# NVlabs/UnseenObjectClustering

Hardware: AMD Instinct MI355X
Metric: frames/sec at 640x480 RGB-D, two-stage clustering (higher is better)
Workload: dtype f32; 1 GPU; configs[3] frames: full two-stage (crop-and-refine) segmentation of single 640x480 RGB-D frames; throughput schedule 3 streams x 4-frame launch sets (one frame at a time: `latency`); frame=640x480, seeds=100, iters=10, crop=224, total_frames=513, frames_per_gpu=513, collective=False, frames_in_flight_per_gpu=12, streams_per_gpu=3, frames_per_launch=4

## Files before the change

### include/uoc_hip.h

```cpp
#ifndef UOC_HIP_H
#define UOC_HIP_H

#include <stddef.h>
#include <stdint.h>

#ifdef __cplusplus
extern "C" {
#endif

#define UOC_OK 0
#define UOC_EINVAL (-22)
#define UOC_ENOMEM (-12)
#define UOC_EHIP (-5)
#define UOC_ENOENT (-2)
#define UOC_ETIMEDOUT (-110)

#define UOC_EMBED_DIM 64
#define UOC_MAX_SEEDS 128
#define UOC_METRIC_COSINE 0
#define UOC_METRIC_EUCLIDEAN 1

int uoc_version(void);
int uoc_is_dev_build(void);
unsigned long long uoc_config_fingerprint(void);
// ... 57 lines not shown

int uoc_net_create(uoc_net **out);
int uoc_net_create_mode(uoc_net **out, int mode);
int uoc_net_embed_dim(const uoc_net *net);
int uoc_net_destroy(uoc_net *net);
int uoc_net_load_param(uoc_net *net, const char *name, const float *host_data, size_t numel);
int uoc_net_finalize(uoc_net *net);
size_t uoc_net_workspace_bytes(const uoc_net *net, int B, int H, int W);
int uoc_net_set_split_precision(uoc_net *net, int on);
int uoc_net_forward(uoc_net *net, const float *d_rgb, const float *d_xyz, int B, int H, int W, float *d_embed,
                    void *d_ws, size_t ws_bytes, void *stream);

#define UOC_CONV_DIRECT 0
#define UOC_CONV_WINOGRAD4 4
#define UOC_CONV_WINOGRAD4_BF16X3 5
int uoc_conv2d_nhwc(const float *d_in, const float *d_w, const float *d_bias, const float *d_res, float *d_out,
                    int G, int B, int H, int W, int Cin, int Cout, int K, int stride, int dil, int pad, int relu,
                    void *stream);
int uoc_conv2d_nhwc_algo(const float *d_in, const float *d_w, const float *d_bias, const float *d_res, float *d_out,
                         int G, int B, int H, int W, int Cin, int Cout, int K, int stride, int dil, int pad, int relu,
                         int algo, void *stream);

int uoc_conv2d_tile_list(int algo, int32_t *out_pairs, int cap);
int uoc_conv2d_nhwc_tile(const float *d_in, const float *d_w, const float *d_bias, const float *d_res, float *d_out,
                         int G, int B, int H, int W, int Cin, int Cout, int K, int stride, int dil, int pad, int relu,
                         int algo, void *stream, int cfg, int bm);
int uoc_conv2d_tile_choice(int G, int B, int H, int W, int Cin, int Cout, int K, int stride, int dil, int algo,
                           int32_t *cfg, int32_t *bm, int32_t *family_bm);
int uoc_net_stem(const float *d_nchw, const float *h_w, const float *h_bias, const float *d_res, int G, int B, int H,
                 int W, int relu, float *d_out, void *stream);
int uoc_maxpool3x3s2_nhwc(const float *d_in, float *d_out, int n_img, int H, int W, int C, void *stream);
int uoc_head(const float *d_fa, const float *d_fb, float *d_embed, int B, int h, int w, int H, int W, int cat,
             void *stream);


typedef struct uoc_roi_table {
  int32_t K;
  int32_t label[128];
  int32_t box[128][4];
} uoc_roi_table;

size_t uoc_roi_workspace_bytes(void);

int uoc_prep_rgbd(const uint8_t *d_bgr, const uint16_t *d_depth_mm, int H, int W, float fx, float fy, float px,
                  float py, float mean_b, float mean_g, float mean_r, float *d_image, float *d_xyz, void *stream);

int uoc_filter_labels_depth(int32_t *d_labels, const float *d_z, long z_batch_stride, int B, int H, int W,
                            float threshold, void *d_ws, size_t ws_bytes, void *stream);

int uoc_roi_build(int32_t *d_labels, const float *d_z, int H, int W, float threshold, float pad_fraction,
                  uoc_roi_table *d_table, void *d_ws, size_t ws_bytes, void *stream);

int uoc_roi_crop(const float *d_rgb, const float *d_xyz, const int32_t *d_labels, int H, int W,
                 const uoc_roi_table *d_table, int K, int S, float *d_rgb_crops, float *d_xyz_crops,
                 float *d_mask_crops, void *stream);

int uoc_roi_match_stats(const int32_t *d_labels_crop, const float *d_mask_crops, const float *d_xyz_crops, int K,
                        int S, int32_t *d_keep, float *d_meanz, void *d_ws, size_t ws_bytes, void *stream);

int uoc_roi_paste(const int32_t *d_labels_crop, const uoc_roi_table *d_table, const int32_t *d_map,
                  const int32_t *d_order, int K, int S, int H, int W, int32_t *d_refined, void *stream);

int uoc_roi_match(const int32_t *d_labels_crop, const float *d_mask_crops, const float *d_xyz_crops,
                  const uoc_roi_table *d_table, int K, int S, int H, int W, int32_t *d_refined, int32_t *d_keep,
                  int32_t *d_plan, int32_t *d_status, void *d_ws, size_t ws_bytes, void *stream);

// ... 253 lines not shown
```

### unseenobjectclustering_amd/_native.py

```python
from __future__ import annotations

import ctypes
import os
from ctypes import c_char_p, c_float, c_int, c_int32, c_long, c_size_t, c_uint32, c_ulonglong, c_void_p, POINTER

from .build import LIB_PATH

_lib = None


class NativeError(RuntimeError):
    pass


P, I, F, Z, L, U = c_void_p, c_int, c_float, c_size_t, c_long, c_uint32
ABI = {
    "uoc_version": (I, []),
    "uoc_is_dev_build": (I, []),
    "uoc_config_fingerprint": (c_ulonglong, []),
    "uoc_shutdown": (I, []),
    "uoc_last_error": (c_char_p, []),
    "uoc_reload_env": (I, []),
    "uoc_ms_set_persistent_fps": (I, [I]),
    "uoc_ms_set_stream_ordering": (I, [I]),
# ... 1 lines not shown
    "uoc_ms_check": (I, [P]),
    "uoc_ms_workspace_bytes": (Z, [I, I, I]),
    "uoc_ms_select_seeds": (I, [P, I, I, I, P, P, P, P, Z, P]),
    "uoc_ms_select_seeds_from": (I, [P, I, I, I, I, P, P, P, P, Z, P]),
    "uoc_ms_hill_climb": (I, [P, I, I, P, I, F, I, P, Z, P]),
    "uoc_ms_seed_components": (I, [P, I, I, F, P, P, P]),
    "uoc_ms_assign": (I, [P, I, I, P, P, P, I, P, P, P, Z, P]),
    "uoc_ms_cluster": (I, [P, I, I, I, F, I, F, P, P, P, P, P, P, Z, P]),
    "uoc_ms_workspace_bytes_wide": (Z, [I, I, I, I]),
    "uoc_ms_cluster_wide": (I, [P, I, I, I, I, F, I, F, P, P, P, P, P, P, Z, P]),
    "uoc_ms_select_seeds_ex": (I, [P, I, I, I, I, P, P, P, I, P, Z, P]),
    "uoc_ms_hill_climb_ex": (I, [P, I, I, P, I, F, I, I, P, Z, P]),
    "uoc_ms_seed_components_ex": (I, [P, I, I, F, I, P, P, P]),
    "uoc_ms_assign_ex": (I, [P, I, I, P, P, P, I, I, P, P, P, Z, P]),
    "uoc_ms_cluster_ex": (I, [P, I, I, I, F, I, F, I, P, P, P, P, P, P, Z, P]),
    "uoc_ms_cluster_wide_ex": (I, [P, I, I, I, I, F, I, F, I, P, P, P, P, P, P, Z, P]),
    "uoc_net_create": (I, [POINTER(P)]),
    "uoc_net_create_mode": (I, [POINTER(P), I]),
    "uoc_net_embed_dim": (I, [P]),
    "uoc_net_destroy": (I, [P]),
    "uoc_net_load_param": (I, [P, c_char_p, P, Z]),
    "uoc_net_finalize": (I, [P]),
    "uoc_net_workspace_bytes": (Z, [P, I, I, I]),
    "uoc_net_set_split_precision": (I, [P, I]),
    "uoc_net_forward": (I, [P, P, P, I, I, I, P, P, Z, P]),
    "uoc_conv2d_nhwc": (I, [P, P, P, P, P, I, I, I, I, I, I, I, I, I, I, I, P]),
    "uoc_conv2d_nhwc_algo": (I, [P, P, P, P, P, I, I, I, I, I, I, I, I, I, I, I, I, P]),
    "uoc_conv2d_tile_list": (I, [I, P, I]),
    "uoc_conv2d_nhwc_tile": (I, [P, P, P, P, P, I, I, I, I, I, I, I, I, I, I, I, I, P, I, I]),
    "uoc_conv2d_tile_choice": (I, [I, I, I, I, I, I, I, I, I, I, P, P, P]),
    "uoc_net_stem": (I, [P, P, P, P, I, I, I, I, I, P, P]),
    "uoc_maxpool3x3s2_nhwc": (I, [P, P, I, I, I, I, P]),
    "uoc_head": (I, [P, P, P, I, I, I, I, I, I, P]),
    "uoc_roi_workspace_bytes": (Z, []),
    "uoc_prep_rgbd": (I, [P, P, I, I, F, F, F, F, F, F, F, P, P, P]),
    "uoc_filter_labels_depth": (I, [P, P, L, I, I, I, F, P, Z, P]),
    "uoc_roi_build": (I, [P, P, I, I, F, F, P, P, Z, P]),
    "uoc_roi_crop": (I, [P, P, P, I, I, P, I, I, P, P, P, P]),
    "uoc_roi_match_stats": (I, [P, P, P, I, I, P, P, P, Z, P]),
    "uoc_roi_paste": (I, [P, P, P, P, I, I, I, I, P, P]),
    "uoc_roi_match": (I, [P, P, P, P, I, I, I, I, P, P, P, P, P, Z, P]),
    "uoc_labels_to_u8": (I, [P, L, P, P, P]),
    "uoc_eval_workspace_bytes": (Z, [I, I]),
    "uoc_eval_pair_stats": (I, [P, P, I, I, I, P, P, Z, P]),
    "uoc_objects_workspace_bytes": (Z, [I, I, I]),
    "uoc_objects": (I, [P, P, P, I, I, I, I, I, P, P, P, P, L, P, P, Z, P]),
    "uoc_track_state_bytes": (Z, [I, I, I]),
    "uoc_track_workspace_bytes": (Z, [I]),
    "uoc_track_reset": (I, [P, I, I, I, I, P]),
    "uoc_track_step": (I, [P, I, I, I, I, I, P, P, P, P, P, Z, P]),
    "uoc_cc_workspace_bytes": (Z, [I, I, I]),
    "uoc_cc_split": (I, [P, I, I, I, I, I, I, P, P, P, P, Z, P]),
    "uoc_plane_workspace_bytes": (Z, [I, I, I, I]),
    "uoc_support_plane": (I, [P, P, I, I, I, I, I, U, P, P, P, P, Z, P]),
    "uoc_planes_workspace_bytes": (Z, [I, I, I, I, I]),
    "uoc_support_planes": (I, [P, P, I, I, I, I, I, I, I, I, U, P, P, P, P, P, P, Z, P]),
    "uoc_relations_workspace_bytes": (Z, [I, I, I]),
    "uoc_relations": (I, [P, P, I, I, I, I, I, I, P, P, P, Z, P]),
    "uoc_placement_workspace_bytes": (Z, [I, I, I, I]),
    "uoc_placement": (I, [P, P, P, I, I, I, I, I, I, I, I, I, P, I, P, P, P, P, P, P, P, Z, P]),
    "uoc_grasp_workspace_bytes": (Z, [I, I, I, I]),
    "uoc_grasp": (I, [P, P, I, I, P, I, I, I, I, I, I, I, P, P, P, Z, P]),
    "uoc_elevation_workspace_bytes": (Z, [I, I, I, I]),
    "uoc_elevation": (I, [P, P, P, I, I, I, I, I, I, I, I, P, I, P, P, P, P, P, P, P, P, P, Z, P]),
    "uoc_footprint_workspace_bytes": (Z, [I, I, I, I]),
    "uoc_footprint": (I, [P, P, P, P, I, I, P, I, P, I, I, P, P, P, P, Z, P]),
# ... 290 lines not shown
```

### unseenobjectclustering_amd/csrc/conv.h

```cpp
#pragma once
#include "common.h"

namespace uoc {

struct ConvParams {
  const float *in;
  const float *w;
  const float *bias;
  const float *res;
  float *out;
  int G, B, H, W, Cin, Ho, Wo, Cout;
  int KH, KW, stride, dil, pad, relu;
  int stem;
  int tune = 1;
  int prof_kc = -1;
  double prof_flops = 0.0;
  int prof_tag[4] = {0, 0, 0, 0};
};

int launch_conv(const ConvParams &p, hipStream_t st);
int conv_tile_list(int *out_pairs, int cap);
int conv_tile_choice(const ConvParams &p, int *cfg, int *bm, int *fam_bm);
int launch_conv_tile(const ConvParams &p, hipStream_t st, int cfg, int bm);

struct W4Tile {
  int bm, bn;
};
int wino4_tile_list(bool split, int *out_pairs, int cap);
void wino4_tile_choice(bool split, int NT, int Cout, int planes, int *bn, int *bm);
int wino4_split_tile_list(int *out_pairs, int cap);
void wino4_split_tile_choice(int NT, int Cout, int planes, int *bn, int *bm);
void wino4_pick_tile(const int (*tiles)[2], int n, int NT, int Cout, int planes, int &bm, int &bn);
int wino4_plane_grid(int NT, int Cout, int planes, int bm, int bn);

bool wino4_eligible(const ConvParams &p);
bool wino4_channels_ok(int Cin, int Cout);
size_t wino4_ws_floats(int G, int B, int H, int W, int d, int Cin, int Cout);
int wino4_num_tiles(int B, int H, int W, int d);
int launch_wino4_weights(const float *w, float *U, int G, int Cout, int Cin, hipStream_t st);
int launch_wino4_conv(const ConvParams &p, const float *U, float *ws, hipStream_t st, const unsigned short *U3 = nullptr,
                      const W4Tile *tile = nullptr);
int launch_wino4_split_weights(const float *U, unsigned short *U3, int G, int Cout, int Cin, hipStream_t st);
int launch_wino4_slice_split(const ConvParams &p0, int Bg, int b0, const unsigned short *U3, float *ws, hipStream_t st,
                             const W4Tile *tile = nullptr);
struct Wino4Geom;
int w4_stage_output(const ConvParams &p, const Wino4Geom &geo, const float *Mw, hipStream_t st);
long wino4_elem_blocks(long items);
int launch_nchw3_to_nhwc4(const float *in, float *out, int B, int H, int W, hipStream_t st);
int launch_maxpool3x3s2(const float *in, float *out, int n_img, int H, int W, int C, int Ho, int Wo, hipStream_t st);
int launch_head(const float *fa, const float *fb, float *embed, int B, int h, int w, int H, int W, int cat,
                hipStream_t st);

}
```

### unseenobjectclustering_amd/csrc/net.hip

```cpp
#include <map>
#include <mutex>
#include <string>
#include <vector>

#include "conv.h"

#include <stdlib.h>

namespace uoc {

struct ConvLayer {
  std::string conv, bn;
  int Cin, Cout, K, stride, dil, pad, relu;
  bool has_bn, has_bias, stem;
  float *d_w = nullptr, *d_b = nullptr;
  float *d_U4 = nullptr;
  unsigned short *d_U3 = nullptr;
  size_t w_per_group = 0;
};

struct Block {
  int conv1, conv2, down;
};

// ... 438 lines not shown
int uoc_conv2d_nhwc_algo(const float *d_in, const float *d_w, const float *d_bias, const float *d_res, float *d_out, int G,
                         int B, int H, int W, int Cin, int Cout, int K, int stride, int dil, int pad, int relu, int algo,
                         void *stream) {
  return conv2d_entry(d_in, d_w, d_bias, d_res, d_out, G, B, H, W, Cin, Cout, K, stride, dil, pad, relu, algo, stream, nullptr);
}

int uoc_conv2d_nhwc_tile(const float *d_in, const float *d_w, const float *d_bias, const float *d_res, float *d_out, int G,
                         int B, int H, int W, int Cin, int Cout, int K, int stride, int dil, int pad, int relu, int algo,
                         void *stream, int cfg, int bm) {
  UOC_REQUIRE(d_in && d_w && d_out, "conv2d tile: null pointer");
  const int tile[2] = {cfg, bm};
  return conv2d_entry(d_in, d_w, d_bias, d_res, d_out, G, B, H, W, Cin, Cout, K, stride, dil, pad, relu, algo, stream, tile);
}

int uoc_conv2d_tile_list(int algo, int32_t *out_pairs, int cap) {
  UOC_REQUIRE(cap >= 0 && (out_pairs || cap == 0), "tile list: null array");
  if (algo == UOC_CONV_DIRECT) return conv_tile_list(out_pairs, cap);
  if (algo == UOC_CONV_WINOGRAD4 || algo == UOC_CONV_WINOGRAD4_BF16X3)
    return wino4_tile_list(algo == UOC_CONV_WINOGRAD4_BF16X3, out_pairs, cap);
  set_error("tile list: unknown algorithm %d", algo);
  return UOC_EINVAL;
}

int uoc_conv2d_tile_choice(int G, int B, int H, int W, int Cin, int Cout, int K, int stride, int dil, int algo, int32_t *cfg,
                           int32_t *bm, int32_t *family_bm) {
  UOC_REQUIRE(cfg && bm, "tile choice: null pointer");
  UOC_REQUIRE(K == 1 || K == 3, "K=%d (only 1 or 3)", K);
  UOC_REQUIRE(G >= 1 && B >= 1 && H >= 1 && W >= 1 && Cin >= 1 && Cout >= 1 && stride >= 1 && dil >= 1, "tile choice: bad shape");
  const ConvParams p = entry_params(G, B, H, W, Cin, Cout, K, stride, dil, K == 3 ? dil : 0, 0);
  if (algo == UOC_CONV_DIRECT) return conv_tile_choice(p, cfg, bm, family_bm);
  if (algo == UOC_CONV_WINOGRAD4 || algo == UOC_CONV_WINOGRAD4_BF16X3) {
    UOC_REQUIRE(wino4_eligible(p), "tile choice: shape not eligible for Winograd F(4x4,3x3)");
    int bn_ = 0, bm_ = 0;
    wino4_tile_choice(algo == UOC_CONV_WINOGRAD4_BF16X3, wino4_num_tiles(B, H, W, dil), Cout, 36 * G, &bn_, &bm_);
    *cfg = bn_;
    *bm = bm_;
    return UOC_OK;
  }
  set_error("tile choice: unknown algorithm %d", algo);
  return UOC_EINVAL;
}

int uoc_net_stem(const float *d_nchw, const float *h_w, const float *h_bias, const float *d_res, int G, int B, int H, int W,
                 int relu, float *d_out, void *stream) {
  UOC_REQUIRE(d_nchw && h_w && d_out, "stem: null pointer");
  UOC_REQUIRE(G >= 1 && B >= 1 && H >= 1 && W >= 1, "stem: bad shape");
  UOC_REQUIRE(d_res == nullptr || d_res != d_out, "stem: the residual must not alias the output");
  UOC_REQUIRE((long)G * B * H * W * 4 < (1l << 31), "stem: input too large");
  hipStream_t st = (hipStream_t)stream;
  const size_t wpg = (size_t)7 * 64 * 32;
  std::vector<float> hw((size_t)G * wpg, 0.f), hb((size_t)G * 64, 0.f);
  const std::vector<double> one(64, 1.0);
  for (int g = 0; g < G; ++g) relayout_weights(h_w + (size_t)g * 64 * 3 * 49, one.data(), 64, 3, 7, true, wpg, hw.data() + g * wpg);
  if (h_bias) hb.assign(h_bias, h_bias + (size_t)G * 64);
  float *d_w = nullptr, *d_b = nullptr, *d_in4 = nullptr;
  int rc = UOC_OK;
  auto run = [&]() -> int {
    UOC_HIP_CHECK(hipMalloc(&d_w, hw.size() * sizeof(float)));
    UOC_HIP_CHECK(hipMalloc(&d_b, hb.size() * sizeof(float)));
    UOC_HIP_CHECK(hipMalloc(&d_in4, (size_t)G * B * H * W * 4 * sizeof(float)));
    UOC_HIP_CHECK(hipMemcpyAsync(d_w, hw.data(), hw.size() * sizeof(float), hipMemcpyHostToDevice, st));
    UOC_HIP_CHECK(hipMemcpyAsync(d_b, hb.data(), hb.size() * sizeof(float), hipMemcpyHostToDevice, st));
    if (int r = launch_nchw3_to_nhwc4(d_nchw, d_in4, G * B, H, W, st)) return r;
    ConvLayer L;
    L.Cin = 3;
    L.Cout = 64;
    L.K = 7;
    L.stride = 2;
    L.dil = 1;
    L.pad = 3;
    L.relu = relu;
    L.has_bn = L.has_bias = false;
    L.stem = true;
    L.d_w = d_w;
// ... 37 lines not shown
```

### unseenobjectclustering_amd/csrc/wino4.hip

```cpp
#include "conv.h"
#include "dma.h"
#include "prof.h"
#include "wino4_math.h"

#include <stdlib.h>

namespace uoc {

constexpr int W4BK = 32;
#ifndef W4_OUT_MIN_BLOCKS
#define W4_OUT_MIN_BLOCKS 2
#endif

__global__ __launch_bounds__(256) void wino4_weight_kernel(const float *__restrict__ w, float *__restrict__ U, int G,
                                                           int Cout, int Cin) {
  const long total = (long)G * Cout * Cin;
  for (long i = (long)blockIdx.x * blockDim.x + threadIdx.x; i < total; i += (long)gridDim.x * blockDim.x) {
    const int ci = (int)(i % Cin);
    const int co = (int)((i / Cin) % Cout);
    const int g = (int)(i / ((long)Cin * Cout));
    wino4_weight_body(w, U, G, Cout, Cin, g, co, ci);
  }
}

template <int VEC>
__global__ __launch_bounds__(256) void wino4_input_kernel(const float *__restrict__ in, float *__restrict__ V,
                                                          Wino4Geom geo, int G, int C) {
  const int CV = C / VEC;
  const long total = (long)G * geo.NT * CV;
#ifndef W4_IN_XCD
#define W4_IN_XCD 1
#endif
  const long vblock = W4_IN_XCD ? (long)(blockIdx.x & 7) * (gridDim.x >> 3) + (blockIdx.x >> 3) : (long)blockIdx.x;
  for (long idx = vblock * blockDim.x + threadIdx.x; idx < total; idx += (long)gridDim.x * blockDim.x) {
    const int cv = (int)(idx % CV);
    const int tau = (int)((idx / CV) % geo.NT);
    const int g = (int)(idx / ((long)CV * geo.NT));
    wino4_input_body<VEC>(in, V, geo, C, g, tau, cv);
  }
}

template <int VEC>
__global__ __launch_bounds__(256, W4_OUT_MIN_BLOCKS) void wino4_output_kernel(const float *__restrict__ M, const float *__restrict__ bias,
                                                           const float *__restrict__ res, float *__restrict__ out,
                                                           Wino4Geom geo, int G, int Cout, int relu) {
  const int CV = Cout / VEC;
  const long total = (long)G * geo.NT * CV;
  for (long idx = (long)blockIdx.x * blockDim.x + threadIdx.x; idx < total; idx += (long)gridDim.x * blockDim.x) {
    const int cv = (int)(idx % CV);
    const int tau = (int)((idx / CV) % geo.NT);
    const int g = (int)(idx / ((long)CV * geo.NT));
    wino4_output_body<VEC>(M, bias, res, out, geo, Cout, relu, g, tau, cv);
  }
}



__device__ __forceinline__ f32x4 w4mfma(float a, float b, f32x4 c) {
  return __builtin_amdgcn_mfma_f32_16x16x4f32(a, b, c, 0, 0, 0);
}

#ifndef UOC_W4_ABLATE
#define UOC_W4_ABLATE 0
#endif
#define W4_BARRIER() do { if (UOC_W4_ABLATE != 1) __builtin_amdgcn_s_barrier(); } while (0)
template <int N>
__device__ __forceinline__ void w4_wait_vmcnt() {
  if (UOC_W4_ABLATE != 2) wait_vmcnt<N>();
}

template <int BM, int BN, bool PAIR, int NW>
__global__ __launch_bounds__(NW * 64) void wino4_gemm_kernel(const float *__restrict__ V, const float *__restrict__ U,
                                                             float *__restrict__ Mo, int NT, int Cin, int Cout, int planes,
                                                             int mtiles, int nt_shift) {
  static_assert(NW == 8 || NW == 4, "waves per block");
  constexpr int WAVES_N = NW / 2;
  constexpr int WM = BM / 2, WN = BN / WAVES_N;
  constexpr int TM = WM / 16, TN = WN / 16;
  constexpr int R = BM + BN;
  constexpr int RPP = NW * 8;
  constexpr int NPA = (BM + RPP - 1) / RPP, NPW = (BN + RPP - 1) / RPP, NPASS = NPA + NPW;
  constexpr int STAGE = R * W4BK;
  static_assert(WM % 16 == 0 && WN % 16 == 0 && R % 8 == 0 && NPASS <= 12, "tile shape");

  extern __shared__ __attribute__((aligned(16))) float smem[];

  const int ntiles = 1 << nt_shift;
  const int per_plane = mtiles << nt_shift;
  const int total = planes * per_plane;
  const int S = (total + 7) >> 3;
  const int xcd = blockIdx.x & 7, jloc = blockIdx.x >> 3, nbl = gridDim.x >> 3;
  const int slice_lo = xcd * S, slice_hi = min(total, slice_lo + S);
  const int first = slice_lo + jloc;
  if (first >= slice_hi) return;
  const int n_items = (slice_hi - first + nbl - 1) / nbl;
  const int cpt = Cin / W4BK;
  const int nchunks = n_items * cpt;

  const unsigned lds_base = (unsigned)(size_t)((__attribute__((address_space(3))) char *)smem);
  const int tid = threadIdx.x, lane = tid & 63;
  const int wave = __builtin_amdgcn_readfirstlane(tid >> 6);
  const int wm = wave / WAVES_N, wn = wave % WAVES_N;
  const int t = lane & 15, q = lane >> 4;

  const unsigned plane_a_bytes = (unsigned)((size_t)NT * Cin * 4), plane_w_bytes = (unsigned)((size_t)Cout * Cin * 4);
  const v4i srd_a = make_srd(V, (unsigned)planes * plane_a_bytes);
  const v4i srd_w = make_srd(U, (unsigned)planes * plane_w_bytes);

  int l_r0[NPASS], l_row[NPASS], l_c4[NPASS];
#pragma unroll
  for (int j = 0; j < NPASS; ++j) {
    const bool isw = j >= NPA;
    int r0 = (isw ? BM + (j - NPA) * RPP : j * RPP) + wave * 8;
    if (!isw && r0 >= BM) r0 = BM - 8;
    if (isw && r0 >= R) r0 = R - 8;
    l_r0[j] = r0;
    const int r = r0 + (lane >> 3);
    l_row[j] = isw ? r - BM : r;
    l_c4[j] = 4 * ((lane & 7) ^ ((r >> 1) & 7));
  }

  int iss_plane, iss_rem, iss_cc = 0;
  {
    iss_plane = first / per_plane;
    iss_rem = first - iss_plane * per_plane;
  }
  unsigned l_voff[NPASS];
  unsigned soff_a, soff_w;
#define W4_ITEM_SETUP()                                                                                  \
  {                                                                                                      \
    const int mt_ = iss_rem >> nt_shift, nt_ = iss_rem & (ntiles - 1);                                   \
    _Pragma("unroll") for (int j = 0; j < NPASS; ++j) {                                                  \
      if (j < NPA) {                                                                                     \
        const int tau_ = min(mt_ * BM + l_row[j], NT - 1);                                               \
        l_voff[j] = (unsigned)((tau_ * Cin + l_c4[j]) * 4);                                              \
      } else {                                                                                           \
        l_voff[j] = (unsigned)(((nt_ * BN + l_row[j]) * Cin + l_c4[j]) * 4);                             \
      }                                                                                                  \
    }                                                                                                    \
    soff_a = (unsigned)__builtin_amdgcn_readfirstlane((int)((unsigned)iss_plane * plane_a_bytes));       \
    soff_w = (unsigned)__builtin_amdgcn_readfirstlane((int)((unsigned)iss_plane * plane_w_bytes));       \
  }
#define W4_ISSUE(STG)                                                                                    \
  {                                                                                                      \
    _Pragma("unroll") for (int j = 0; j < NPASS; ++j) {                                                  \
      const unsigned dst_ = lds_base + (unsigned)(((STG)*STAGE + l_r0[j] * W4BK) * sizeof(float));       \
      if (UOC_W4_ABLATE == 4) continue;                                                                  \
      if (j < NPA)                                                                                       \
        blds16(srd_a, l_voff[j], soff_a, dst_);                                                          \
      else                                                                                               \
        blds16(srd_w, l_voff[j], soff_w, dst_);                                                          \
    }                                                                                                    \
  }
#define W4_ADVANCE()                                                                                     \
  {                                                                                                      \
    if (++iss_cc == cpt) {                                                                               \
      iss_cc = 0;                                                                                        \
      iss_rem += nbl;                                                                                    \
      while (iss_rem >= per_plane) {                                                                     \
        iss_rem -= per_plane;                                                                            \
        ++iss_plane;                                                                                     \
      }                                                                                                  \
      W4_ITEM_SETUP()                                                                                    \
    } else {                                                                                             \
      soff_a += W4BK * 4;                                                                                \
      soff_w += W4BK * 4;                                                                                \
    }                                                                                                    \
  }
#define W4_FRAG(STG, HH, WA, XB)                                                                         \
  {                                                                                                      \
    const float *base_ = smem + (STG)*STAGE;                                                             \
    const int slot_ = ((4 * (HH) + q) ^ ((t >> 1) & 7)) * 4;                                             \
    _Pragma("unroll") for (int j = 0; j < TN; ++j) WA[j] =                                               \
        *reinterpret_cast<const float4 *>(base_ + (BM + wn * WN + 16 * j + t) * W4BK + slot_);           \
    _Pragma("unroll") for (int i = 0; i < TM; ++i) XB[i] =                                               \
        *reinterpret_cast<const float4 *>(base_ + (wm * WM + 16 * i + t) * W4BK + slot_);                \
  }
#define W4_MFMA_E(WA, XB, E)                                                                                   \
  {                                                                                                            \
    _Pragma("unroll") for (int j = 0; j < TN; ++j) _Pragma("unroll") for (int i = 0; i < TM; ++i) acc[j][i] =  \
        w4mfma(WA[j].E, XB[i].E, acc[j][i]);                                                                   \
  }

  f32x4 acc[TN][TM];
#pragma unroll
  for (int j = 0; j < TN; ++j)
#pragma unroll
    for (int i = 0; i < TM; ++i) acc[j][i] = f32x4{0.f, 0.f, 0.f, 0.f};

  int cmp_plane = iss_plane, cmp_rem = iss_rem, cmp_cc = 0;

  float4 wa0[TN], xb0[TM], wa1[TN], xb1[TM];
  const bool early = NW == 4 || wave < 4;
  auto epilogue = [&]() {
    cmp_cc = 0;
    const int mt = cmp_rem >> nt_shift, nt = cmp_rem & (ntiles - 1);
    float *dst = Mo + (size_t)cmp_plane * NT * Cout;
#pragma unroll
    for (int j = 0; j < TN; ++j) {
      const int co = nt * BN + wn * WN + 16 * j + 4 * q;
#pragma unroll
      for (int i = 0; i < TM; ++i) {
        const int m = mt * BM + wm * WM + 16 * i + t;
        if (m < NT)
          *reinterpret_cast<float4 *>(dst + (size_t)m * Cout + co) =
              make_float4(acc[j][i][0], acc[j][i][1], acc[j][i][2], acc[j][i][3]);
        acc[j][i] = f32x4{0.f, 0.f, 0.f, 0.f};
      }
    }
    cmp_rem += nbl;
    while (cmp_rem >= per_plane) {
      cmp_rem -= per_plane;
      ++cmp_plane;
    }
  };
  if constexpr (PAIR) {
    W4_ITEM_SETUP()
    W4_ISSUE(0)
    W4_ADVANCE()
    W4_ISSUE(1)
    W4_ADVANCE()
    w4_wait_vmcnt<0>();
    W4_BARRIER();
    W4_FRAG(0, 0, wa0, xb0)
    if (NW == 8 && wave >= 4) __builtin_amdgcn_s_setprio(1);
    for (int kc = 0; kc < nchunks; kc += 2) {
      const int sa = (kc & 2), sb = sa + 1, sc = sa ^ 2, sd = sc + 1;
      const bool more = kc + 2 < nchunks;
      if (more && early) {
        W4_ISSUE(sc)
        W4_ADVANCE()
        W4_ISSUE(sd)
        W4_ADVANCE()
      }
      W4_MFMA_E(wa0, xb0, x)
      W4_FRAG(sa, 1, wa1, xb1)
      __builtin_amdgcn_sched_barrier(0);
      W4_MFMA_E(wa0, xb0, y)
      W4_MFMA_E(wa0, xb0, z)
      W4_MFMA_E(wa0, xb0, w)
      if (more && !early) {
        W4_ISSUE(sc)
        W4_ADVANCE()
        W4_ISSUE(sd)
// ... 54 lines not shown
    W4_MFMA_E(wa0, xb0, z)
    W4_MFMA_E(wa0, xb0, w)
    if (kc + 2 < nchunks && !early) W4_ISSUE(s_nn)
    if (kc + 2 < nchunks) W4_ADVANCE()
    if (kc + 2 < nchunks)
      w4_wait_vmcnt<NPASS>();
    else
      w4_wait_vmcnt<0>();
    __builtin_amdgcn_s_waitcnt(0xC07F);
    W4_BARRIER();
    if (kc + 1 < nchunks) W4_FRAG(s_nxt, 0, wa0, xb0)
    __builtin_amdgcn_sched_barrier(0);
    W4_MFMA_E(wa1, xb1, x)
    W4_MFMA_E(wa1, xb1, y)
    W4_MFMA_E(wa1, xb1, z)
    W4_MFMA_E(wa1, xb1, w)
    __builtin_amdgcn_sched_barrier(0);
    __builtin_amdgcn_s_waitcnt(0xC07F);
    __builtin_amdgcn_sched_barrier(0);
    if (++cmp_cc == cpt) epilogue();
    const int tmp = s_cur;
    s_cur = s_nxt;
    s_nxt = s_nn;
    s_nn = tmp;
  }
#undef W4_ITEM_SETUP
#undef W4_ISSUE
#undef W4_ADVANCE
#undef W4_FRAG
#undef W4_MFMA_E
}

template <int BM, int BN, bool PAIR, int NW>
static int launch_wino4_gemm_t(const float *V, const float *U, float *Mo, int NT, int Cin, int Cout, int planes, int nblocks,
                               hipStream_t st) {
  const int mtiles = (NT + BM - 1) / BM, ntiles = Cout / BN;
  int nt_shift = 0;
  while ((1 << nt_shift) < ntiles) ++nt_shift;
  UOC_REQUIRE((1 << nt_shift) == ntiles, "winograd F(4x4): Cout / %d = %d is not a power of two", BN, ntiles);
  constexpr int NSTAGE = PAIR ? 4 : 3;
  const size_t lds = (size_t)NSTAGE * (BM + BN) * W4BK * sizeof(float);
  static_assert((size_t)NSTAGE * (BM + BN) * W4BK * sizeof(float) <= 160 * 1024, "LDS ring too large");
  UOC_REQUIRE(!PAIR || (Cin / W4BK) % 2 == 0, "winograd F(4x4): the pair loop needs an even number of 32-channel chunks");
  static DeviceOnce attr_set;
  if (int rc = opt_in_dynamic_lds(reinterpret_cast<const void *>(&wino4_gemm_kernel<BM, BN, PAIR, NW>), lds, attr_set)) return rc;
  hipLaunchKernelGGL((wino4_gemm_kernel<BM, BN, PAIR, NW>), dim3(nblocks), dim3(NW * 64), lds, st, V, U, Mo, NT, Cin, Cout, planes,
                     mtiles, nt_shift);
  UOC_LAUNCH_CHECK();
  return UOC_OK;
}

#define UOC_W4_TILES(X) \
  X(96, 128) X(128, 128) X(160, 128) X(192, 128) X(96, 64) X(128, 64) X(160, 64) X(192, 64)
static const int kW4Tiles[][2] = {
#define X(A, B) {A, B},
    UOC_W4_TILES(X)
#undef X
};

static int plane_per_xcd() {
  const int dev = device_num_cu(), ncu = dev > 0 ? dev : 256;
  return ncu / 8 > 0 ? ncu / 8 : 1;
}

void wino4_pick_tile(const int (*tiles)[2], int n, int NT, int Cout, int planes, int &bm, int &bn) {
  const int per_xcd = plane_per_xcd();
  double best = -1;
  for (int i = 0; i < n; ++i) {
    const int BM = tiles[i][0], BN = tiles[i][1];
    if (Cout % BN) continue;
    const long items = (long)planes * ((NT + BM - 1) / BM) * (Cout / BN);
    const long S = (items + 7) / 8;
    const long steps = (S + per_xcd - 1) / per_xcd;
    const double cost = (double)steps * BM * BN * (1.0 + 0.05 * (192.0 / BM - 1.0)) * (BN == 64 ? 1.06 : 1.0);
    if (best < 0 || cost < best) {
      best = cost;
      bm = BM;
      bn = BN;
    }
  }
}

int wino4_plane_grid(int NT, int Cout, int planes, int bm, int bn) {
  const int per_xcd = plane_per_xcd();
  const long items = (long)planes * ((NT + bm - 1) / bm) * (Cout / bn);
  const long S = (items + 7) / 8;
  return 8 * (int)(S < per_xcd ? S : per_xcd);
}

static int launch_wino4_gemm(const float *V, const float *U, float *Mo, int NT, int Cin, int Cout, int planes, hipStream_t st,
                             const W4Tile *tile) {
  int bm = 160, bn = Cout % 128 == 0 ? 128 : 64;
  if (tile) {
    bm = tile->bm;
    bn = tile->bn;
    UOC_REQUIRE((bn == 64 || bn == 128) && Cout % bn == 0, "winograd F(4x4): Cout=%d does not admit BN=%d", Cout, bn);
  } else {
    wino4_pick_tile(kW4Tiles, (int)(sizeof(kW4Tiles) / sizeof(kW4Tiles[0])), NT, Cout, planes, bm, bn);
  }
  const int nblocks = wino4_plane_grid(NT, Cout, planes, bm, bn);
  const int cpt = Cin / W4BK;
  const bool pair = cpt % 2 == 0 && cpt >= 4;
#define X(A, B)                                                                                                      \
  if (bm == A && bn == B)                                                                                            \
    return pair ? launch_wino4_gemm_t<A, B, true, 8>(V, U, Mo, NT, Cin, Cout, planes, nblocks, st)                    \
                : launch_wino4_gemm_t<A, B, false, 8>(V, U, Mo, NT, Cin, Cout, planes, nblocks, st);
  UOC_W4_TILES(X)
#undef X
  set_error("winograd F(4x4): no GEMM tile %dx%d", bm, bn);
  return UOC_EINVAL;
}

int wino4_tile_list(bool split, int *out_pairs, int cap) {
  if (split) return wino4_split_tile_list(out_pairs, cap);
  const int n = (int)(sizeof(kW4Tiles) / sizeof(kW4Tiles[0]));
  for (int i = 0; i < n && i < cap && out_pairs; ++i) {
    out_pairs[2 * i] = kW4Tiles[i][1];
    out_pairs[2 * i + 1] = kW4Tiles[i][0];
  }
  return n;
}

void wino4_tile_choice(bool split, int NT, int Cout, int planes, int *bn, int *bm) {
  if (split) return wino4_split_tile_choice(NT, Cout, planes, bn, bm);
  *bm = 160;
  *bn = Cout % 128 == 0 ? 128 : 64;
  wino4_pick_tile(kW4Tiles, (int)(sizeof(kW4Tiles) / sizeof(kW4Tiles[0])), NT, Cout, planes, *bm, *bn);
}

bool wino4_channels_ok(int Cin, int Cout) {
  const int n64 = Cout / 64;
  return Cin % W4BK == 0 && Cout % 64 == 0 && n64 > 0 && (n64 & (n64 - 1)) == 0;
}

bool wino4_eligible(const ConvParams &p) {
  return !p.stem && p.KH == 3 && p.KW == 3 && p.stride == 1 && p.pad == p.dil && wino4_channels_ok(p.Cin, p.Cout) &&
         p.Ho == p.H && p.Wo == p.W;
}

int wino4_num_tiles(int B, int H, int W, int d) { return make_geom4(B, H, W, d).NT; }

size_t wino4_ws_floats(int G, int B, int H, int W, int d, int Cin, int Cout) {
  const Wino4Geom geo = make_geom4(B, H, W, d);
  return (size_t)G * 36 * geo.NT * 5 / 2 * (size_t)(Cin > Cout ? Cin : Cout) + 64;
}

int launch_wino4_weights(const float *w, float *U, int G, int Cout, int Cin, hipStream_t st) {
  const long total = (long)G * Cout * Cin;
  long blocks = (total + 255) / 256;
  if (blocks > 4096) blocks = 4096;
  hipLaunchKernelGGL(wino4_weight_kernel, dim3((unsigned)blocks), dim3(256), 0, st, w, U, G, Cout, Cin);
  UOC_LAUNCH_CHECK();
  return UOC_OK;
}

long wino4_elem_blocks(long items) {
  long blocks = (items + 255) / 256;
  const long cap = 16384;
  blocks = blocks < cap ? blocks : cap;
  return (blocks + 7) / 8 * 8;
// ... 76 lines not shown
```

Before: 175.3 frames/s.

## Split Winograd F(4x4) GEMM tail wave into smaller sub-tiles to fill XCDs

Adds a cost-modelled plan that runs full waves of Winograd GEMM tiles with the normal tile size, then splits the leftover items on each XCD into 2 or 4 smaller sub-tiles so the last wave uses more CUs. By default the full and tail phases are fused into one kernel, with a __syncthreads between them. A global knob can force the part count or request two separate launches. Tile selection now takes Cin into account through the new cost model. The risks are extra template instantiations, the smaller tail tiles being less efficient, and the cost model's constants possibly choosing badly.

```diff
diff --git a/include/uoc_hip.h b/include/uoc_hip.h
--- a/include/uoc_hip.h
+++ b/include/uoc_hip.h
@@ -113,6 +113,7 @@
 int uoc_maxpool3x3s2_nhwc(const float *d_in, float *d_out, int n_img, int H, int W, int C, void *stream);
 int uoc_head(const float *d_fa, const float *d_fb, float *d_embed, int B, int h, int w, int H, int W, int cat,
              void *stream);
+int uoc_w4_set_parts(int parts, int two_launches);
 
 
 typedef struct uoc_roi_table {
diff --git a/unseenobjectclustering_amd/_native.py b/unseenobjectclustering_amd/_native.py
--- a/unseenobjectclustering_amd/_native.py
+++ b/unseenobjectclustering_amd/_native.py
@@ -57,6 +57,7 @@
     "uoc_net_stem": (I, [P, P, P, P, I, I, I, I, I, P, P]),
     "uoc_maxpool3x3s2_nhwc": (I, [P, P, I, I, I, I, P]),
     "uoc_head": (I, [P, P, P, I, I, I, I, I, I, P]),
+    "uoc_w4_set_parts": (I, [I, I]),
     "uoc_roi_workspace_bytes": (Z, []),
     "uoc_prep_rgbd": (I, [P, P, I, I, F, F, F, F, F, F, F, P, P, P]),
     "uoc_filter_labels_depth": (I, [P, P, L, I, I, I, F, P, Z, P]),
diff --git a/unseenobjectclustering_amd/csrc/conv.h b/unseenobjectclustering_amd/csrc/conv.h
--- a/unseenobjectclustering_amd/csrc/conv.h
+++ b/unseenobjectclustering_amd/csrc/conv.h
@@ -27,10 +27,11 @@
   int bm, bn;
 };
 int wino4_tile_list(bool split, int *out_pairs, int cap);
-void wino4_tile_choice(bool split, int NT, int Cout, int planes, int *bn, int *bm);
+void wino4_tile_choice(bool split, int NT, int Cin, int Cout, int planes, int *bn, int *bm);
+int wino4_set_parts(int parts, int two_launches);
 int wino4_split_tile_list(int *out_pairs, int cap);
 void wino4_split_tile_choice(int NT, int Cout, int planes, int *bn, int *bm);
-void wino4_pick_tile(const int (*tiles)[2], int n, int NT, int Cout, int planes, int &bm, int &bn);
+void wino4_pick_tile(const int (*tiles)[2], int n, int NT, int Cout, int planes, int &bm, int &bn, int Cin = 0, int force_parts = 1);
 int wino4_plane_grid(int NT, int Cout, int planes, int bm, int bn);
 
 bool wino4_eligible(const ConvParams &p);
diff --git a/unseenobjectclustering_amd/csrc/net.hip b/unseenobjectclustering_amd/csrc/net.hip
--- a/unseenobjectclustering_amd/csrc/net.hip
+++ b/unseenobjectclustering_amd/csrc/net.hip
@@ -494,7 +494,7 @@
   if (algo == UOC_CONV_WINOGRAD4 || algo == UOC_CONV_WINOGRAD4_BF16X3) {
     UOC_REQUIRE(wino4_eligible(p), "tile choice: shape not eligible for Winograd F(4x4,3x3)");
     int bn_ = 0, bm_ = 0;
-    wino4_tile_choice(algo == UOC_CONV_WINOGRAD4_BF16X3, wino4_num_tiles(B, H, W, dil), Cout, 36 * G, &bn_, &bm_);
+    wino4_tile_choice(algo == UOC_CONV_WINOGRAD4_BF16X3, wino4_num_tiles(B, H, W, dil), Cin, Cout, 36 * G, &bn_, &bm_);
     *cfg = bn_;
     *bm = bm_;
     return UOC_OK;
@@ -502,6 +502,8 @@
   set_error("tile choice: unknown algorithm %d", algo);
   return UOC_EINVAL;
 }
+
+int uoc_w4_set_parts(int parts, int two_launches) { return wino4_set_parts(parts, two_launches); }
 
 int uoc_net_stem(const float *d_nchw, const float *h_w, const float *h_bias, const float *d_res, int G, int B, int H, int W,
                  int relu, float *d_out, void *stream) {
diff --git a/unseenobjectclustering_amd/csrc/w4_plan.h b/unseenobjectclustering_amd/csrc/w4_plan.h
--- /dev/null
+++ b/unseenobjectclustering_amd/csrc/w4_plan.h
@@ -0,0 +1,102 @@
+#pragma once
+
+#if defined(__HIPCC__)
+#define UOC_W4_HD __host__ __device__
+#else
+#define UOC_W4_HD
+#endif
+
+namespace uoc {
+
+struct W4Plan {
+  int bm, bn;
+  int mtiles, nt_shift;
+  int per_xcd;
+  int total, S;
+  int full;
+  int parts;
+  int pm_shift, pn_shift;
+  int grid_full;
+  int grid_tail;
+  double cost;
+};
+
+UOC_W4_HD inline void w4_slice(int total, int S, int xcd, int &lo, int &hi) {
+  lo = xcd * S;
+  hi = lo + S < total ? lo + S : total;
+  if (lo > hi) lo = hi;
+}
+
+UOC_W4_HD inline void w4_tail_unit(int u, int tail_lo, int per_plane, int nt_shift, int pm_shift, int pn_shift, int bm2, int bn2,
+                                   int &plane, int &row0, int &col0) {
+  const int item = tail_lo + (u >> (pm_shift + pn_shift));
+  const int part = u & ((1 << (pm_shift + pn_shift)) - 1);
+  plane = item / per_plane;
+  const int rem = item - plane * per_plane;
+  const int mt = rem >> nt_shift, nt = rem & ((1 << nt_shift) - 1);
+  row0 = ((mt << pm_shift) + (part >> pn_shift)) * bm2;
+  col0 = ((nt << pn_shift) + (part & ((1 << pn_shift) - 1))) * bn2;
+}
+
+inline double w4_tile_cost(int bm, int bn) { return (double)bm * bn * (1.0 + 0.05 * (192.0 / bm - 1.0)) * (bn == 64 ? 1.06 : 1.0); }
+constexpr double W4_COST_TAIL_FIXED = 22000.0;
+constexpr double W4_COST_PART = 1.0;
+constexpr double W4_COST_MARGIN = 1.03;
+
+inline double w4_plan_cost(const W4Plan &p, int Cin) {
+  const int cpt = Cin / 32 > 0 ? Cin / 32 : 1;
+  if (p.parts == 1) return (double)((p.S + p.per_xcd - 1) / p.per_xcd) * w4_tile_cost(p.bm, p.bn);
+  const double c = (double)(p.full / p.per_xcd) * w4_tile_cost(p.bm, p.bn);
+  const int units = (p.S - p.full) * p.parts, nbl = p.grid_tail / 8;
+  const int rounds = (units + nbl - 1) / nbl;
+  return W4_COST_MARGIN * (c + rounds * W4_COST_PART * w4_tile_cost(p.bm >> p.pm_shift, p.bn >> p.pn_shift) + W4_COST_TAIL_FIXED / cpt);
+}
+
+inline bool w4_split_shape(int bm, int bn, int P, int &pm_shift, int &pn_shift) {
+  pm_shift = pn_shift = 0;
+  if (P == 1) return true;
+  const bool half_m = bm == 192 || bm == 128;
+  if (P == 2) {
+    if (bn == 128) return pn_shift = 1, true;
+    if (half_m) return pm_shift = 1, true;
+    return false;
+  }
+  if (P == 4 && bn == 128 && half_m) return pm_shift = pn_shift = 1, true;
+  return false;
+}
+
+inline W4Plan w4_make_plan(int NT, int Cin, int Cout, int planes, int ncu, int bm, int bn, int force) {
+  W4Plan w = {};
+  w.bm = bm;
+  w.bn = bn;
+  w.mtiles = (NT + bm - 1) / bm;
+  const int ntiles = Cout / bn;
+  while ((1 << w.nt_shift) < ntiles) ++w.nt_shift;
+  w.per_xcd = ncu / 8 > 0 ? ncu / 8 : 1;
+  w.total = planes * w.mtiles * ntiles;
+  w.S = (w.total + 7) / 8;
+  w.full = w.S;
+  w.parts = 1;
+  w.grid_full = 8 * (w.S < w.per_xcd ? w.S : w.per_xcd);
+  w.grid_tail = 0;
+  w.cost = w4_plan_cost(w, Cin);
+  if (force == 1) return w;
+  W4Plan best = w;
+  const int full = w.S / w.per_xcd * w.per_xcd, left = w.S - full;
+  if (left == 0) return w;
+  for (int P = 2; P <= 4; P += 2) {
+    if (force > 1 && force != P) continue;
+    W4Plan c = w;
+    if (!w4_split_shape(bm, bn, P, c.pm_shift, c.pn_shift)) continue;
+    c.parts = P;
+    c.full = full;
+    c.grid_full = full > 0 ? 8 * c.per_xcd : 0;
+    const int units = left * P;
+    c.grid_tail = 8 * (units < c.per_xcd ? units : c.per_xcd);
+    c.cost = w4_plan_cost(c, Cin);
+    if (force > 1 || c.cost < best.cost) best = c;
+  }
+  return best;
+}
+
+}
diff --git a/unseenobjectclustering_amd/csrc/wino4.hip b/unseenobjectclustering_amd/csrc/wino4.hip
--- a/unseenobjectclustering_amd/csrc/wino4.hip
+++ b/unseenobjectclustering_amd/csrc/wino4.hip
@@ -1,9 +1,11 @@
 #include "conv.h"
 #include "dma.h"
 #include "prof.h"
+#include "w4_plan.h"
 #include "wino4_math.h"
 
 #include <stdlib.h>
+#include <atomic>
 
 namespace uoc {
 
@@ -69,10 +71,10 @@
   if (UOC_W4_ABLATE != 2) wait_vmcnt<N>();
 }
 
-template <int BM, int BN, bool PAIR, int NW>
-__global__ __launch_bounds__(NW * 64) void wino4_gemm_kernel(const float *__restrict__ V, const float *__restrict__ U,
-                                                             float *__restrict__ Mo, int NT, int Cin, int Cout, int planes,
-                                                             int mtiles, int nt_shift) {
+template <int BM, int BN, bool PAIR, int NW, bool TAIL>
+__device__ __forceinline__ void w4_gemm_body(const float *__restrict__ V, const float *__restrict__ U, float *__restrict__ Mo,
+                                             int NT, int Cin, int Cout, int planes, int mtiles, int nt_shift, int full,
+                                             int pm_shift, int pn_shift) {
   static_assert(NW == 8 || NW == 4, "waves per block");
   constexpr int WAVES_N = NW / 2;
   constexpr int WM = BM / 2, WN = BN / WAVES_N;
@@ -90,7 +92,9 @@
   const int total = planes * per_plane;
   const int S = (total + 7) >> 3;
   const int xcd = blockIdx.x & 7, jloc = blockIdx.x >> 3, nbl = gridDim.x >> 3;
-  const int slice_lo = xcd * S, slice_hi = min(total, slice_lo + S);
+  const int tail_lo = min(total, xcd * S + full);
+  const int slice_lo = TAIL ? 0 : xcd * S;
+  const int slice_hi = TAIL ? max(0, min(total, xcd * S + S) - tail_lo) << (pm_shift + pn_shift) : min(min(total, slice_lo + S), slice_lo + full);
   const int first = slice_lo + jloc;
   if (first >= slice_hi) return;
   const int n_items = (slice_hi - first + nbl - 1) / nbl;
@@ -121,7 +125,10 @@
   }
 
   int iss_plane, iss_rem, iss_cc = 0;
-  {
+  if constexpr (TAIL) {
+    iss_plane = 0;
+    iss_rem = first;
+  } else {
     iss_plane = first / per_plane;
     iss_rem = first - iss_plane * per_plane;
   }
@@ -129,13 +136,14 @@
   unsigned soff_a, soff_w;
 #define W4_ITEM_SETUP()                                                                                  \
   {                                                                                                      \
-    const int mt_ = iss_rem >> nt_shift, nt_ = iss_rem & (ntiles - 1);                                   \
+    int row0_ = (iss_rem >> nt_shift) * BM, col0_ = (iss_rem & (ntiles - 1)) * BN;                       \
+    if constexpr (TAIL) w4_tail_unit(iss_rem, tail_lo, per_plane, nt_shift, pm_shift, pn_shift, BM, BN, iss_plane, row0_, col0_); \
     _Pragma("unroll") for (int j = 0; j < NPASS; ++j) {                                                  \
       if (j < NPA) {                                                                                     \
-        const int tau_ = min(mt_ * BM + l_row[j], NT - 1);                                               \
+        const int tau_ = min(row0_ + l_row[j], NT - 1);                                                  \
         l_voff[j] = (unsigned)((tau_ * Cin + l_c4[j]) * 4);                                              \
       } else {                                                                                           \
-        l_voff[j] = (unsigned)(((nt_ * BN + l_row[j]) * Cin + l_c4[j]) * 4);                             \
+        l_voff[j] = (unsigned)(((col0_ + l_row[j]) * Cin + l_c4[j]) * 4);                                \
       }                                                                                                  \
     }                                                                                                    \
     soff_a = (unsigned)__builtin_amdgcn_readfirstlane((int)((unsigned)iss_plane * plane_a_bytes));       \
@@ -157,7 +165,7 @@
     if (++iss_cc == cpt) {                                                                               \
       iss_cc = 0;                                                                                        \
       iss_rem += nbl;                                                                                    \
-      while (iss_rem >= per_plane) {                                                                     \
+      while (!TAIL && iss_rem >= per_plane) {                                                            \
         iss_rem -= per_plane;                                                                            \
         ++iss_plane;                                                                                     \
       }                                                                                                  \
@@ -194,14 +202,15 @@
   const bool early = NW == 4 || wave < 4;
   auto epilogue = [&]() {
     cmp_cc = 0;
-    const int mt = cmp_rem >> nt_shift, nt = cmp_rem & (ntiles - 1);
+    int row0 = (cmp_rem >> nt_shift) * BM, col0 = (cmp_rem & (ntiles - 1)) * BN;
+    if constexpr (TAIL) w4_tail_unit(cmp_rem, tail_lo, per_plane, nt_shift, pm_shift, pn_shift, BM, BN, cmp_plane, row0, col0);
     float *dst = Mo + (size_t)cmp_plane * NT * Cout;
 #pragma unroll
     for (int j = 0; j < TN; ++j) {
-      const int co = nt * BN + wn * WN + 16 * j + 4 * q;
+      const int co = col0 + wn * WN + 16 * j + 4 * q;
 #pragma unroll
       for (int i = 0; i < TM; ++i) {
-        const int m = mt * BM + wm * WM + 16 * i + t;
+        const int m = row0 + wm * WM + 16 * i + t;
         if (m < NT)
           *reinterpret_cast<float4 *>(dst + (size_t)m * Cout + co) =
               make_float4(acc[j][i][0], acc[j][i][1], acc[j][i][2], acc[j][i][3]);
@@ -209,7 +218,7 @@
       }
     }
     cmp_rem += nbl;
-    while (cmp_rem >= per_plane) {
+    while (!TAIL && cmp_rem >= per_plane) {
       cmp_rem -= per_plane;
       ++cmp_plane;
     }
@@ -330,26 +339,79 @@
 }
 
 template <int BM, int BN, bool PAIR, int NW>
-static int launch_wino4_gemm_t(const float *V, const float *U, float *Mo, int NT, int Cin, int Cout, int planes, int nblocks,
-                               hipStream_t st) {
-  const int mtiles = (NT + BM - 1) / BM, ntiles = Cout / BN;
-  int nt_shift = 0;
-  while ((1 << nt_shift) < ntiles) ++nt_shift;
-  UOC_REQUIRE((1 << nt_shift) == ntiles, "winograd F(4x4): Cout / %d = %d is not a power of two", BN, ntiles);
-  constexpr int NSTAGE = PAIR ? 4 : 3;
-  const size_t lds = (size_t)NSTAGE * (BM + BN) * W4BK * sizeof(float);
-  static_assert((size_t)NSTAGE * (BM + BN) * W4BK * sizeof(float) <= 160 * 1024, "LDS ring too large");
-  UOC_REQUIRE(!PAIR || (Cin / W4BK) % 2 == 0, "winograd F(4x4): the pair loop needs an even number of 32-channel chunks");
+__global__ __launch_bounds__(NW * 64) void wino4_gemm_kernel(const float *__restrict__ V, const float *__restrict__ U,
+                                                             float *__restrict__ Mo, int NT, int Cin, int Cout, int planes,
+                                                             int mtiles, int nt_shift, int full) {
+  w4_gemm_body<BM, BN, PAIR, NW, false>(V, U, Mo, NT, Cin, Cout, planes, mtiles, nt_shift, full, 0, 0);
+}
+
+template <int BM, int BN, bool PAIR>
+__global__ __launch_bounds__(512) void wino4_gemm_tail_kernel(const float *__restrict__ V, const float *__restrict__ U,
+                                                              float *__restrict__ Mo, int NT, int Cin, int Cout, int planes,
+                                                              int mtiles, int nt_shift, int full, int pm_shift, int pn_shift) {
+  w4_gemm_body<BM, BN, PAIR, 8, true>(V, U, Mo, NT, Cin, Cout, planes, mtiles, nt_shift, full, pm_shift, pn_shift);
+}
+
+template <int BM, int BN, int PMS, int PNS, bool PAIR>
+__global__ __launch_bounds__(512) void wino4_gemm_parts_kernel(const float *__restrict__ V, const float *__restrict__ U,
+                                                               float *__restrict__ Mo, int NT, int Cin, int Cout, int planes,
+                                                               int mtiles, int nt_shift, int full) {
+  w4_gemm_body<BM, BN, PAIR, 8, false>(V, U, Mo, NT, Cin, Cout, planes, mtiles, nt_shift, full, 0, 0);
+  __syncthreads();
+  w4_gemm_body<(BM >> PMS), (BN >> PNS), PAIR, 8, true>(V, U, Mo, NT, Cin, Cout, planes, mtiles, nt_shift, full, PMS, PNS);
+}
+
+struct W4Args {
+  const float *V, *U;
+  float *Mo;
+  int NT, Cin, Cout, planes;
+};
+
+template <int BM, int BN, bool PAIR>
+constexpr size_t w4_lds_bytes() {
+  constexpr size_t lds = (size_t)(PAIR ? 4 : 3) * (BM + BN) * W4BK * sizeof(float);
+  static_assert(lds <= 160 * 1024, "LDS ring too large");
+  return lds;
+}
+
+template <int BM, int BN, bool PAIR, int NW>
+static int launch_wino4_gemm_t(const W4Args &a, const W4Plan &plan, hipStream_t st) {
+  constexpr size_t lds = w4_lds_bytes<BM, BN, PAIR>();
   static DeviceOnce attr_set;
   if (int rc = opt_in_dynamic_lds(reinterpret_cast<const void *>(&wino4_gemm_kernel<BM, BN, PAIR, NW>), lds, attr_set)) return rc;
-  hipLaunchKernelGGL((wino4_gemm_kernel<BM, BN, PAIR, NW>), dim3(nblocks), dim3(NW * 64), lds, st, V, U, Mo, NT, Cin, Cout, planes,
-                     mtiles, nt_shift);
+  hipLaunchKernelGGL((wino4_gemm_kernel<BM, BN, PAIR, NW>), dim3(plan.grid_full), dim3(NW * 64), lds, st, a.V, a.U, a.Mo, a.NT, a.Cin,
+                     a.Cout, a.planes, plan.mtiles, plan.nt_shift, plan.full);
   UOC_LAUNCH_CHECK();
   return UOC_OK;
 }
 
+template <int BM, int BN, bool PAIR>
+static int launch_wino4_tail_t(const W4Args &a, const W4Plan &plan, hipStream_t st) {
+  constexpr size_t lds = w4_lds_bytes<BM, BN, PAIR>();
+  static DeviceOnce attr_set;
+  if (int rc = opt_in_dynamic_lds(reinterpret_cast<const void *>(&wino4_gemm_tail_kernel<BM, BN, PAIR>), lds, attr_set)) return rc;
+  hipLaunchKernelGGL((wino4_gemm_tail_kernel<BM, BN, PAIR>), dim3(plan.grid_tail), dim3(512), lds, st, a.V, a.U, a.Mo, a.NT, a.Cin, a.Cout,
+                     a.planes, plan.mtiles, plan.nt_shift, plan.full, plan.pm_shift, plan.pn_shift);
+  UOC_LAUNCH_CHECK();
+  return UOC_OK;
+}
+
+template <int BM, int BN, int PMS, int PNS, bool PAIR>
+static int launch_wino4_parts_t(const W4Args &a, const W4Plan &plan, hipStream_t st) {
+  constexpr size_t lds = w4_lds_bytes<BM, BN, PAIR>();
+  static DeviceOnce attr_set;
+  if (int rc = opt_in_dynamic_lds(reinterpret_cast<const void *>(&wino4_gemm_parts_kernel<BM, BN, PMS, PNS, PAIR>), lds, attr_set)) return rc;
+  hipLaunchKernelGGL((wino4_gemm_parts_kernel<BM, BN, PMS, PNS, PAIR>), dim3(plan.grid_full), dim3(512), lds, st, a.V, a.U, a.Mo, a.NT,
+                     a.Cin, a.Cout, a.planes, plan.mtiles, plan.nt_shift, plan.full);
+  UOC_LAUNCH_CHECK();
+  return UOC_OK;
+}
+
 #define UOC_W4_TILES(X) \
   X(96, 128) X(128, 128) X(160, 128) X(192, 128) X(96, 64) X(128, 64) X(160, 64) X(192, 64)
+#define UOC_W4_PART_TILES(X) X(96, 64) X(128, 64) X(160, 64) X(192, 64) X(64, 64)
+#define UOC_W4_SPLITS(X) \
+  X(96, 128, 0, 1) X(128, 128, 0, 1) X(160, 128, 0, 1) X(192, 128, 0, 1) X(128, 128, 1, 1) X(192, 128, 1, 1) X(128, 64, 1, 0) X(192, 64, 1, 0)
 static const int kW4Tiles[][2] = {
 #define X(A, B) {A, B},
     UOC_W4_TILES(X)
@@ -361,16 +423,21 @@
   return ncu / 8 > 0 ? ncu / 8 : 1;
 }
 
-void wino4_pick_tile(const int (*tiles)[2], int n, int NT, int Cout, int planes, int &bm, int &bn) {
-  const int per_xcd = plane_per_xcd();
+static std::atomic<int> g_w4_parts{0}, g_w4_two_launches{0};
+int wino4_set_parts(int parts, int two_launches) {
+  UOC_REQUIRE(parts == 0 || parts == 1 || parts == 2 || parts == 4, "winograd F(4x4): parts = %d (0, 1, 2 or 4)", parts);
+  g_w4_parts.store(parts);
+  g_w4_two_launches.store(two_launches != 0);
+  return UOC_OK;
+}
+
+void wino4_pick_tile(const int (*tiles)[2], int n, int NT, int Cout, int planes, int &bm, int &bn, int Cin, int force_parts) {
+  const int ncu = 8 * plane_per_xcd();
   double best = -1;
   for (int i = 0; i < n; ++i) {
     const int BM = tiles[i][0], BN = tiles[i][1];
     if (Cout % BN) continue;
-    const long items = (long)planes * ((NT + BM - 1) / BM) * (Cout / BN);
-    const long S = (items + 7) / 8;
-    const long steps = (S + per_xcd - 1) / per_xcd;
-    const double cost = (double)steps * BM * BN * (1.0 + 0.05 * (192.0 / BM - 1.0)) * (BN == 64 ? 1.06 : 1.0);
+    const double cost = w4_make_plan(NT, Cin > 0 ? Cin : W4BK, Cout, planes, ncu, BM, BN, Cin > 0 ? force_parts : 1).cost;
     if (best < 0 || cost < best) {
       best = cost;
       bm = BM;
@@ -380,32 +447,53 @@
 }
 
 int wino4_plane_grid(int NT, int Cout, int planes, int bm, int bn) {
-  const int per_xcd = plane_per_xcd();
-  const long items = (long)planes * ((NT + bm - 1) / bm) * (Cout / bn);
-  const long S = (items + 7) / 8;
-  return 8 * (int)(S < per_xcd ? S : per_xcd);
+  return w4_make_plan(NT, W4BK, Cout, planes, 8 * plane_per_xcd(), bm, bn, 1).grid_full;
 }
 
 static int launch_wino4_gemm(const float *V, const float *U, float *Mo, int NT, int Cin, int Cout, int planes, hipStream_t st,
                              const W4Tile *tile) {
   int bm = 160, bn = Cout % 128 == 0 ? 128 : 64;
+  const int force = g_w4_parts.load();
   if (tile) {
     bm = tile->bm;
     bn = tile->bn;
     UOC_REQUIRE((bn == 64 || bn == 128) && Cout % bn == 0, "winograd F(4x4): Cout=%d does not admit BN=%d", Cout, bn);
   } else {
-    wino4_pick_tile(kW4Tiles, (int)(sizeof(kW4Tiles) / sizeof(kW4Tiles[0])), NT, Cout, planes, bm, bn);
-  }
-  const int nblocks = wino4_plane_grid(NT, Cout, planes, bm, bn);
+    wino4_pick_tile(kW4Tiles, (int)(sizeof(kW4Tiles) / sizeof(kW4Tiles[0])), NT, Cout, planes, bm, bn, Cin, force);
+  }
+  UOC_REQUIRE(Cout / bn > 0 && (Cout / bn & (Cout / bn - 1)) == 0, "winograd F(4x4): Cout / %d = %d is not a power of two", bn, Cout / bn);
+  const W4Plan plan = w4_make_plan(NT, Cin, Cout, planes, 8 * plane_per_xcd(), bm, bn, force);
+  const W4Args a = {V, U, Mo, NT, Cin, Cout, planes};
   const int cpt = Cin / W4BK;
   const bool pair = cpt % 2 == 0 && cpt >= 4;
+  if (plan.parts > 1 && plan.full > 0 && !g_w4_two_launches.load()) {
+#define X(A, B, PMS, PNS)                                                                  \
+  if (bm == A && bn == B && plan.pm_shift == PMS && plan.pn_shift == PNS)                  \
+    return pair ? launch_wino4_parts_t<A, B, PMS, PNS, true>(a, plan, st) : launch_wino4_parts_t<A, B, PMS, PNS, false>(a, plan, st);
+    UOC_W4_SPLITS(X)
+#undef X
+    set_error("winograd F(4x4): no GEMM tile %dx%d in %d parts", bm, bn, plan.parts);
+    return UOC_EINVAL;
+  }
+  if (plan.full > 0) {
+    int rc = UOC_EINVAL;
+    bool found = false;
 #define X(A, B)                                                                                                      \
-  if (bm == A && bn == B)                                                                                            \
-    return pair ? launch_wino4_gemm_t<A, B, true, 8>(V, U, Mo, NT, Cin, Cout, planes, nblocks, st)                    \
-                : launch_wino4_gemm_t<A, B, false, 8>(V, U, Mo, NT, Cin, Cout, planes, nblocks, st);
-  UOC_W4_TILES(X)
+  if (!found && bm == A && bn == B) {                                                                                \
+    found = true;                                                                                                    \
+    rc = pair ? launch_wino4_gemm_t<A, B, true, 8>(a, plan, st) : launch_wino4_gemm_t<A, B, false, 8>(a, plan, st);  \
+  }
+    UOC_W4_TILES(X)
 #undef X
-  set_error("winograd F(4x4): no GEMM tile %dx%d", bm, bn);
+    if (!found) set_error("winograd F(4x4): no GEMM tile %dx%d", bm, bn);
+    if (rc || plan.parts == 1) return rc;
+  }
+  const int bm2 = bm >> plan.pm_shift, bn2 = bn >> plan.pn_shift;
+#define X(A, B) \
+  if (bm2 == A && bn2 == B) return pair ? launch_wino4_tail_t<A, B, true>(a, plan, st) : launch_wino4_tail_t<A, B, false>(a, plan, st);
+  UOC_W4_PART_TILES(X)
+#undef X
+  set_error("winograd F(4x4): no part tile %dx%d", bm2, bn2);
   return UOC_EINVAL;
 }
 
@@ -419,11 +507,11 @@
   return n;
 }
 
-void wino4_tile_choice(bool split, int NT, int Cout, int planes, int *bn, int *bm) {
+void wino4_tile_choice(bool split, int NT, int Cin, int Cout, int planes, int *bn, int *bm) {
   if (split) return wino4_split_tile_choice(NT, Cout, planes, bn, bm);
   *bm = 160;
   *bn = Cout % 128 == 0 ? 128 : 64;
-  wino4_pick_tile(kW4Tiles, (int)(sizeof(kW4Tiles) / sizeof(kW4Tiles[0])), NT, Cout, planes, *bm, *bn);
+  wino4_pick_tile(kW4Tiles, (int)(sizeof(kW4Tiles) / sizeof(kW4Tiles[0])), NT, Cout, planes, *bm, *bn, Cin, g_w4_parts.load());
 }
 
 bool wino4_channels_ok(int Cin, int Cout) {
```

New measurement: 175.3 frames/s (median of 3 runs). About the same (+0.0%).
